# myfavouritekk/vdetlib

Measured on AMD Instinct MI355X. Metric: boxes/sec whole-node (NMS+temporal-conv+link), 300f×10k-box synth; mAP parity, higher is better.
Workload: dtype f32; 1 GPU; configs[1]+[2]: 1 video/GPU, 300 frames x 10000 boxes x 200 classes; per-(frame,class) NMS thresh 0.30 + temporal max-pool w=3 + 3-tap temporal convolution; greedy tubelets: 10 tracks/class (stop < 0.90), IoU-link >= 0.50, spatial max-pool IoU > 0.70 + completion + temporal max-pool; frames=300, boxes=10000, classes=200, scores=rand, parallelism=video-per-gpu x1, 4 distinct videos in flight per GPU

## Files before the change

### vdetlib_amd/csrc/adjrows_kernels.hpp

```cpp
#pragma once
#include <hip/hip_runtime.h>
#include <stdint.h>

#include "nms_kernels.hpp"
#include "binsort_kernels.hpp"

namespace vdet {

constexpr int kRowsChunk = 16;
constexpr int kRowsStage = 8192;
constexpr int kRowsStride = 72;

__global__ __launch_bounds__(256) void strip_totals_kernel(const GroupDesc *__restrict__ groups, const TileDesc *__restrict__ tiles,
                                                           int nstrips, const uint32_t *__restrict__ row_deg,
                                                           const uint32_t *__restrict__ group_flags, uint32_t *__restrict__ totals)
{
    const int lane = threadIdx.x & 63;
    const int sidx = blockIdx.x * 4 + (int)(threadIdx.x >> 6);
    if (sidx >= nstrips) return;
    const TileDesc td = tiles[sidx >> 2];
    const GroupDesc gd = groups[td.group];
    const int v = (td.row_tile * (kRowsPerTile / 64) + (sidx & 3)) * 64 + lane;
    uint32_t t = 0u;
    if ((group_flags[td.group] & kFlagRegular) && v < gd.nbox) t = (row_deg[gd.box_off + v] + 7u) & ~7u;
// ... 116 lines not shown
    const uint32_t total = s_total;
    const bool staged = total <= (uint32_t)kRowsStage;
    uint16_t *slab = adj + s_base;
    constexpr int kRowsSuper = 4 * kRowsChunk;
    for (int s0 = 0; s0 < ne; s0 += kRowsSuper) {
        unsigned long long mw[4 * WPW];
        uint16_t xw[4 * WPW];
#pragma unroll
        for (int j = 0; j < 4 * WPW; ++j) {
            const int q = j / WPW, i = j % WPW;
            const int c = (int)scol[min(s0 + kRowsChunk * q + w + 4 * i, ne - 1)];
            mw[j] = gbits[bit_word(B, min(v, B - 1), c)];
            xw[j] = tr[min(c * 64 + lane, B - 1)];
        }
#pragma unroll
        for (int q = 0; q < 4; ++q) {
            const int e0 = s0 + kRowsChunk * q;
            if (e0 >= ne) break;
#pragma unroll
            for (int i = 0; i < WPW; ++i) {
                const int el = w + 4 * i;
                sb[el * kRowsStride + lane] = (e0 + el < ne && v < B) ? mw[q * WPW + i] : 0ull;
                sx[el * 64 + lane] = xw[q * WPW + i];
            }
            lds_only_barrier();
#pragma unroll 1
            for (int i = 0; i < kRowsChunk / 4; ++i) {
                const int el = 4 * i + xa;
                unsigned long long m = sb[el * kRowsStride + xrow];
                const uint32_t cnt = (uint32_t)__popcll(m);
                if (__ballot(cnt != 0u) == 0ull) continue;
                const uint16_t *sxw = sx + el * 64;
                uint32_t pos = 0u;
                if (cnt != 0u) {
                    const uint32_t at = atomicAdd(&scur[xrow], cnt);
                    if (at == 0u) spad[xrow] = sxw[__ffsll(m) - 1];
                    pos = my_off + at;
                }
                if (staged) {
                    while (__ballot(m != 0ull) != 0ull) {
                        if (m != 0ull) {
                            const unsigned long long m1 = m & (m - 1ull);
                            const uint16_t v0 = sxw[__ffsll(m) - 1];
                            const uint16_t v1 = sxw[m1 ? __ffsll(m1) - 1 : 0];
                            sstage[pos] = v0;
                            if (m1) sstage[pos + 1] = v1;
                            pos += m1 ? 2u : 1u;
                            m = m1 & (m1 - 1ull);
                        }
                    }
                } else {
                    while (__ballot(m != 0ull) != 0ull) {
                        if (m != 0ull) {
                            slab[pos++] = sxw[__ffsll(m) - 1];
                            m &= m - 1ull;
                        }
                    }
                }
            }
            lds_only_barrier();
        }
    }
    __syncthreads();
    if (tid < 64) {
        const uint32_t deg = srow_deg[tid];
        const uint32_t p = srow_off[tid] + deg, padv = spad[tid];
        const uint32_t npad = ((deg + 7u) & ~7u) - deg;
        if (deg != 0u)
            for (uint32_t k = 0; k < npad; ++k) { if (staged) sstage[p + k] = (uint16_t)padv; else slab[p + k] = (uint16_t)padv; }
    }
    if (staged) {
        __syncthreads();
        const uint4 *s4 = reinterpret_cast<const uint4 *>(sstage);
        uint4 *d4 = reinterpret_cast<uint4 *>(slab);
        for (uint32_t i = tid; i < (total >> 3); i += 256) d4[i] = s4[i];
    }
}

__global__ __launch_bounds__(256) void adj_finish_kernel(const GroupDesc *__restrict__ groups, const TileDesc *__restrict__ tiles,
                                                         const uint32_t *__restrict__ row_deg, uint2 *__restrict__ row_meta,
                                                         uint16_t *__restrict__ adj, uint32_t slot_cap, int *__restrict__ status,
                                                         const uint32_t *__restrict__ group_flags, const float4 *__restrict__ xbox_all,
                                                         const uint16_t *__restrict__ xord_all, int over_bits,
                                                         WalkMeta *__restrict__ wmeta, uint4 *__restrict__ wmeta16)
{
    const TileDesc td = tiles[blockIdx.x];
    const uint32_t gf = group_flags[td.group];
    if (!(gf & kFlagRegular)) return;
    const GroupDesc gd = groups[td.group];
    const int v = td.row_tile * kRowsPerTile + (int)threadIdx.x;
    if (v >= gd.nbox) return;
    const uint32_t row = (uint32_t)(gd.box_off + v);
    const uint32_t deg = row_deg[row];
    const int vo = (int)xord_all[row];
    const float4 bx = xbox_all[row];
    const bool over = deg > slot_cap;
    if (over) atomicOr(status, over_bits);
    const uint32_t p = over ? 0u : row * slot_cap;
    const uint32_t d = over ? 0u : deg;
    if (d & 7u) {
        uint16_t *l = adj + (uint64_t)p;
        for (uint32_t k = d; k < ((d + 7u) & ~7u); ++k) l[k] = (uint16_t)vo;
    }
    row_meta[gd.box_off + vo] = make_uint2(p, d);
    const bool rec16 = wmeta16 && (gf & kFlagU16);
    if (wmeta && !rec16) {
        wmeta[gd.box_off + vo].box = over ? make_float4(0.f, 0.f, 0.f, 0.f) : bx;
        wmeta[gd.box_off + vo].row = make_uint4(p, d, 0u, 0u);
    }
    if (rec16)
        wmeta16[gd.box_off + vo] = over ? make_uint4(0u, 0u, 0u, 0u)
                                        : make_uint4((uint32_t)bx.x | ((uint32_t)bx.y << 16), (uint32_t)bx.z | ((uint32_t)bx.w << 16), p, d);
}

__global__ __launch_bounds__(256) void deg_sum_kernel(const uint32_t *__restrict__ row_deg, int64_t n, unsigned long long *__restrict__ out)
{
    unsigned long long s = 0ull;
    for (int64_t i = (int64_t)blockIdx.x * 256 + threadIdx.x; i < n; i += (int64_t)gridDim.x * 256) s += (row_deg[i] + 7u) & ~7u;
    for (int d = 32; d > 0; d >>= 1) s += __shfl_xor(s, d, 64);
    if ((threadIdx.x & 63) == 0 && s) atomicAdd(out, s);
}

__global__ void pool_start_kernel(unsigned long long *pool_used, unsigned long long first) { *pool_used = first; }

}
```

### vdetlib_amd/csrc/graphlists_kernels.hpp

```cpp
#pragma once
#include <hip/hip_runtime.h>
#include <stdint.h>

#include "nms_kernels.hpp"

namespace vdet {

__device__ __forceinline__ int qreach_slot(const GroupDesc &gd, int g) { return ((gd.box_off >> 8) + g) * 4; }

__global__ __launch_bounds__(256) void row_classes_kernel(const float4 *__restrict__ xbox, const GroupDesc *__restrict__ groups,
                                                          const uint32_t *__restrict__ group_flags, float one_minus_t,
                                                          uint16_t *__restrict__ rowperm, float *__restrict__ qreach)
{
    __shared__ float sw[256];
    __shared__ float sreach[256];
    const int g = blockIdx.x, t = blockIdx.y, tid = threadIdx.x;
    if (!(group_flags[g] & kFlagRegular)) return;
    const GroupDesc gd = groups[g];
    if (t * 256 >= gd.nbox) return;
    const int s = t * 256 + tid;
    const bool valid = s < gd.nbox;
    float wd = 3.0e38f, reach = -3.0e38f;
    if (valid) { const float4 b = xbox[gd.box_off + s]; wd = b.z - b.x; reach = b.x + one_minus_t * ((b.z - b.x) + 1.0f) * 1.001f + 1.0f; }
    sw[tid] = wd;
    __syncthreads();
    int rank = 0;
    for (int j = 0; j < 256; ++j) { const float o = sw[j]; rank += (o < wd || (o == wd && j < tid)) ? 1 : 0; }
    if (valid) rowperm[gd.box_off + t * 256 + rank] = (uint16_t)s;
    sreach[rank] = reach;
    __syncthreads();
    float rc = sreach[tid];
#pragma unroll
    for (int d = 32; d > 0; d >>= 1) rc = fmaxf(rc, __shfl_xor(rc, d, 64));
    if ((tid & 63) == 0) qreach[qreach_slot(gd, g) + 4 * t + (tid >> 6)] = rc;
}

struct ListItem { int32_t group; int32_t tq; };

struct GraphListsParams {
    const float4 *xbox;
    const uint16_t *xord;
    const GroupDesc *groups;
    const uint32_t *group_flags;
    const ListItem *items;
    int nitems;
    float t32, hg, one_minus_t;
    uint32_t *row_deg;
    const float2 *reach_table;
    const uint16_t *rowperm;
    const float *qreach;
    uint16_t *adj;
    uint32_t slot_cap;
    int *status;
    int over_bits;
    uint32_t trash_off;
};

__device__ __forceinline__ void emit_half(uint16_t *__restrict__ adj, uint32_t h, uint32_t boff, const uint16_t *ids, uint32_t *lpos,
                                          const uint16_t myid)
{
    constexpr int kSlots = 4;
    if (__ballot(h != 0u) == 0ull) return;
    uint32_t hk[kSlots];
    uint16_t ek[kSlots];
    int bk[kSlots];
#pragma unroll
    for (int k = 0; k < kSlots; ++k) { hk[k] = h; bk[k] = __builtin_ctz(h | 0x80000000u); h &= h - 1u; }
#pragma unroll
    for (int k = 0; k < kSlots; ++k) ek[k] = ids[bk[k]];
#pragma unroll
    for (int k = 0; k < kSlots; ++k) {
        if (hk[k] != 0u) {
            *reinterpret_cast<uint16_t *>(reinterpret_cast<char *>(adj) + (boff + 2u * k)) = ek[k];
            const uint32_t o = __hip_atomic_fetch_add(&lpos[bk[k]], 2u, __ATOMIC_RELAXED, __HIP_MEMORY_SCOPE_WAVEFRONT);
            *reinterpret_cast<uint16_t *>(reinterpret_cast<char *>(adj) + o) = myid;
        }
    }
    boff += 2u * kSlots;
    while (__ballot(h != 0u) != 0ull) {
        if (h != 0u) {
            const int b = __builtin_ctz(h);
            *reinterpret_cast<uint16_t *>(reinterpret_cast<char *>(adj) + boff) = ids[b];
            const uint32_t o = __hip_atomic_fetch_add(&lpos[b], 2u, __ATOMIC_RELAXED, __HIP_MEMORY_SCOPE_WAVEFRONT);
            *reinterpret_cast<uint16_t *>(reinterpret_cast<char *>(adj) + o) = myid;
            boff += 2u;
            h &= h - 1u;
        }
    }
}

__device__ __forceinline__ void emit_block(const uint32_t slot_cap, uint16_t *__restrict__ adj, int *__restrict__ status, const int over_bits,
                                           const uint32_t trash_off, unsigned long long m, const uint32_t tcnt, const uint32_t pat,
                                           const uint32_t ptat, const uint32_t row_slot, const uint32_t col_slot, const uint16_t *cids,
                                           const uint16_t myid, uint32_t *lpos, const int lane)
{
    const uint32_t cnt = (uint32_t)__popcll(m);
    const bool rover = pat + cnt > slot_cap, cover = ptat + tcnt > slot_cap;
    if ((rover && cnt) || (cover && tcnt)) atomicOr(status, over_bits);
    lpos[lane] = cover ? trash_off : (col_slot * slot_cap + ptat) * 2u;
    const uint32_t boff = rover ? trash_off : (row_slot * slot_cap + pat) * 2u;
    emit_half(adj, (uint32_t)m, boff, cids, lpos, myid);
    emit_half(adj, (uint32_t)(m >> 32), boff + 2u * (uint32_t)__popc((uint32_t)m), cids + 32, lpos + 32, myid);
}

template <bool XS, bool INTS>
__device__ __forceinline__ void margin_block(const float4 brx, const float rarea, const float4 *sb, const float *sa, float t32, float hg,
                                             uint32_t &lo, uint32_t &hi)
{
    uint32_t nr0 = 0, nr1 = 0;
#pragma unroll 1
    for (int g = 0; g < 4; ++g) {
#pragma unroll
        for (int j = 0; j < 8; ++j) {
            const int k = 31 - 8 * g - j;
// ... 119 lines not shown
```

### vdetlib_amd/csrc/nms_kernels.hpp

```cpp
#pragma once
#include <hip/hip_runtime.h>
#include <stdint.h>

namespace vdet {

struct GroupDesc {
    int32_t box_off;
    int32_t nbox;
    int64_t bits_off;
};

__device__ __host__ __forceinline__ int64_t bit_word(int nbox, int v, int c)
{
    const int W = (nbox + 63) >> 6;
    return ((int64_t)(v >> 6) * W + c) * 64 + (v & 63);
}
__host__ __device__ __forceinline__ int64_t bit_words_of_group(int nbox)
{
    const int64_t W = (nbox + 63) >> 6;
    return W * W * 64;
}

struct TileDesc {
    int32_t group;
// ... 64 lines not shown
    if (group_flags && (group_flags[td.group] & kFlagRegular)) return;
    const GroupDesc gd = groups[td.group];
    const int B = gd.nbox;
    const int tid = threadIdx.x;
    const int v = td.row_tile * kRowsPerTile + tid;
    const int W = (B + 63) >> 6;
    int wper = (W + gridDim.y - 1) / gridDim.y;
    wper = (wper + 3) & ~3;
    const int w0 = blockIdx.y * wper;
    const int w1 = min(W, w0 + wper);
    if (w0 >= w1) return;

    const float qnan = __uint_as_float(0x7FC00000u);
    float4 brow = make_float4(qnan, qnan, qnan, qnan);
    if (v < B) brow = boxes[gd.box_off + v];
    const float rarea = box_area(brow);
    uint32_t zcnt = 0;

    for (int wt = w0; wt < w1; wt += 4) {
        __syncthreads();
        {
            const int u = wt * 64 + tid;
            float4 bi = make_float4(qnan, qnan, qnan, qnan);
            if (u < B) bi = boxes[gd.box_off + u];
            sbox[tid] = bi;
            sarea[tid] = box_area(bi);
        }
        __syncthreads();
        const int nw = min(4, w1 - wt);
        for (int q = 0; q < nw; ++q) {
            uint32_t lo = 0, hi = 0;
#pragma unroll
            for (int k = 0; k < 32; ++k) {
                const uint32_t p = pair_pred(brow, rarea, sbox[q * 64 + k], sarea[q * 64 + k], t32);
                lo |= (p & 1u) << k;
                zcnt += p >> 1;
            }
#pragma unroll
            for (int k = 0; k < 32; ++k) {
                const uint32_t p = pair_pred(brow, rarea, sbox[q * 64 + 32 + k], sarea[q * 64 + 32 + k], t32);
                hi |= (p & 1u) << k;
                zcnt += p >> 1;
            }
            uint64_t m = ((uint64_t)hi << 32) | lo;
            const int cbase = (wt + q) * 64;
            if (v >= cbase && v < cbase + 64) {
                m &= ~(1ull << (v - cbase));
                const uint32_t ps = pair_pred(brow, rarea, brow, rarea, t32);
                zcnt -= ps >> 1;
            }
            if (v < B) bits[gd.bits_off + bit_word(B, v, wt + q)] = m;
        }
    }
    if (v < B && zcnt) {
        atomicAdd(&row_z[gd.box_off + v], zcnt);
        group_z[td.group] = 1u;
    }
}

struct FrameIndex {
    const float4 *xbox;
    const uint16_t *xord;
    const uint32_t *cum;
    const float *info;
    const uint2 *xbox16;
    const uint16_t *xord16;
    int64_t bias16;
};

__device__ __host__ __forceinline__ int64_t pair_pos(int64_t box_off_plus_g) { return (box_off_plus_g + 1) & ~(int64_t)1; }

__device__ __forceinline__ int xbucket(float x, float xmin, float scale)
{
    const float t = (x - xmin) * scale;
    return t <= 0.0f ? 0 : (t >= 255.0f ? 255 : (int)t);
}

__global__ void xkey_kernel(const float4 *__restrict__ boxes, uint32_t *__restrict__ keys, int64_t n)
{
    const int64_t i = (int64_t)blockIdx.x * blockDim.x + threadIdx.x;
    if (i < n) keys[i] = ~score_key(boxes[i].x);
}

__global__ __launch_bounds__(256) void frame_index_kernel(const float4 *__restrict__ boxes, const GroupDesc *__restrict__ groups,
                                                          const uint16_t *__restrict__ xord_all, float4 *__restrict__ xbox_all,
                                                          uint32_t *__restrict__ cum, float *__restrict__ info,
                                                          const uint32_t *__restrict__ group_flags, uint2 *__restrict__ xbox16,
                                                          uint16_t *__restrict__ xord16)
{
    __shared__ float smin[256], smax[256], swm[256];
    __shared__ uint32_t hist[257];
    const int f = blockIdx.x, tid = threadIdx.x;
    const int B = groups[f].nbox;
    const int64_t fo = groups[f].box_off;
    const float4 *fb = boxes + fo;
    const uint16_t *xord = xord_all + fo;
    float4 *xbox = xbox_all + fo;
    float mn = 3.0e38f, mx = -3.0e38f, wm = 0.0f;
    const bool u16 = xbox16 && (group_flags[f] & kFlagU16);
    const int64_t p16 = pair_pos(fo + f);
    for (int r = tid; r < B; r += 256) {
        const uint16_t o = xord[r];
        const float4 b = fb[o];
        xbox[r] = b;
        if (u16) {
            xbox16[p16 + r] = make_uint2((uint32_t)b.x | ((uint32_t)b.y << 16), (uint32_t)b.z | ((uint32_t)b.w << 16));
            xord16[p16 + r] = o;
        }
        mn = fminf(mn, b.x); mx = fmaxf(mx, b.x); wm = fmaxf(wm, (b.z - b.x) + 1.0f);
    }
    smin[tid] = mn; smax[tid] = mx; swm[tid] = wm;
    for (int i = tid; i < 257; i += 256) hist[i] = 0;
    __syncthreads();
    for (int d = 128; d > 0; d >>= 1) {
        if (tid < d) { smin[tid] = fminf(smin[tid], smin[tid + d]); smax[tid] = fmaxf(smax[tid], smax[tid + d]); swm[tid] = fmaxf(swm[tid], swm[tid + d]); }
        __syncthreads();
    }
    const float xmin = smin[0], xmax = smax[0];
    const float scale = xmax > xmin ? 256.0f / (xmax - xmin) : 0.0f;
    for (int r = tid; r < B; r += 256) atomicAdd(&hist[xbucket(fb[r].x, xmin, scale) + 1], 1u);
    __syncthreads();
    if (tid == 0) {
        uint32_t run = 0;
        for (int k = 0; k <= 256; ++k) { run += hist[k]; cum[(int64_t)f * 257 + k] = run; }
        info[f * 4 + 0] = xmin; info[f * 4 + 1] = scale; info[f * 4 + 2] = swm[0]; info[f * 4 + 3] = 0.0f;
    }
}

__device__ __forceinline__ void xwindow(const FrameIndex &ix, int f, float x1c, float wc, double t, int &r0, int &r1)
{
    const float xmin = ix.info[f * 4 + 0], scale = ix.info[f * 4 + 1], wmax = ix.info[f * 4 + 2];
    const double wj = fmin((double)wmax, (double)wc / t * 1.001);
    const double lo = (double)x1c - (1.0 - t) * wj * 1.001 - 1.0;
    const double hi = (double)x1c + (1.0 - t) * (double)wc * 1.001 + 1.0;
    const int b0 = xbucket((float)fmax(lo, -3.0e38), xmin, scale);
    const int b1 = xbucket((float)fmin(hi, 3.0e38), xmin, scale);
    r0 = (int)ix.cum[(int64_t)f * 257 + b0];
    r1 = (int)ix.cum[(int64_t)f * 257 + b1 + 1];
}

constexpr float kRegularCoordMax = 1152921504606846976.0f;
__global__ __launch_bounds__(256) void frame_flags_kernel(const float4 *__restrict__ boxes,
                                                          const GroupDesc *__restrict__ groups,
                                                          uint32_t *__restrict__ group_flags,
                                                          int *__restrict__ n_irregular)
{
    const GroupDesc gd = groups[blockIdx.x];
    int bad = 0, wide = 0;
    const float inf = __uint_as_float(0x7F800000u);
    for (int v = threadIdx.x; v < gd.nbox; v += 256) {
        const float4 b = boxes[gd.box_off + v];
        const float w = (b.z - b.x) + 1.0f, h = (b.w - b.y) + 1.0f;
        const float a = w * h;
        const bool ok = fabsf(b.x) <= kRegularCoordMax && fabsf(b.y) <= kRegularCoordMax && fabsf(b.z) <= kRegularCoordMax &&
                        fabsf(b.w) <= kRegularCoordMax && w > 0.0f && h > 0.0f && a < inf;
        bad |= ok ? 0 : 1;
        const bool small = b.x == truncf(b.x) && b.y == truncf(b.y) && b.z == truncf(b.z) && b.w == truncf(b.w) &&
                           fmaxf(fmaxf(b.x, b.y), fmaxf(b.z, b.w)) <= 65535.0f &&
                           ((__float_as_uint(b.x) | __float_as_uint(b.y) | __float_as_uint(b.z) | __float_as_uint(b.w)) >> 31) == 0u;
        wide |= small ? 0 : 1;
    }
    const int any_bad = __syncthreads_or(bad);
    const int any_wide = __syncthreads_or(wide);
    if (threadIdx.x == 0) {
        group_flags[blockIdx.x] = (any_bad ? 0u : kFlagRegular) | (any_wide ? 0u : kFlagU16);
        if (any_bad) atomicAdd(n_irregular, 1);
    }
}

__device__ __attribute__((noinline)) bool pair_pred_exact_slow(float4 bi, float iarea, float4 bj, float jarea, float t32)
{
    return (pair_pred(bi, iarea, bj, jarea, t32) & 1u) != 0;
}

struct TilePair {
    int32_t group;
    int16_t rt, ct;
};

__device__ __forceinline__ float amax(float a, float b) { float r; asm("v_max_f32 %0, %1, %2" : "=v"(r) : "v"(a), "v"(b)); return r; }
__device__ __forceinline__ float amin(float a, float b) { float r; asm("v_min_f32 %0, %1, %2" : "=v"(r) : "v"(a), "v"(b)); return r; }

template <bool XSORTED = false>
__device__ __forceinline__ bool pred_regular(float4 br, float rarea, float4 bc, float carea, float t32, float t32e,
                                             bool &border)
{
    const float xx1 = XSORTED ? bc.x : amax(br.x, bc.x);
    const float yy1 = amax(br.y, bc.y);
    const float xx2 = amin(br.z, bc.z);
    const float yy2 = amin(br.w, bc.w);
    const float w = amax(0.0f, (xx2 - xx1) + 1.0f);
    const float h = (yy2 - yy1) + 1.0f;
    const float inter = w * h;
    const float uni = (rarea + carea) - inter;
    const float r = __builtin_fmaf(-t32, uni, inter);
    const float bnd = t32e * uni;
    const bool p = r >= 0.0f;
    border = !p && (r >= -bnd);
    return p;
}

__device__ __forceinline__ void shl1_or_sign(uint32_t &acc, float v)
{
    acc = __builtin_amdgcn_alignbit(acc, __float_as_uint(v), 31);
}

template <bool XSORTED, bool INTS>
// ... 1400 lines not shown
```

### vdetlib_amd/csrc/vdet_capi.hip

```cpp
#include <hip/hip_runtime.h>
#include <atomic>
#include <chrono>

#include <algorithm>
#include <cmath>
#include <cstdarg>
#include <cstdio>
#include <cstdlib>
#include <cstring>
#include <initializer_list>
#include <string>
#include <vector>

#include "../../include/vdet_hip.h"
#include "nms_kernels.hpp"
#include "binsort_kernels.hpp"
#include "small_kernels.hpp"
#include "detnms_kernels.hpp"
#include "fused_kernels.hpp"
#include "adjrows_kernels.hpp"
#include "graphlists_kernels.hpp"
#include "temporal_kernels.hpp"
#include "tubelet_kernels.hpp"
#include "track_kernels.hpp"
// ... 354 lines not shown
    while (p < x) p <<= 1;
    return p;
}

int translate_status(vdet_ctx *c, int st)
{
    if (st & kStPoolAsync) return fail(c, VDET_EAGAIN, "adjacency pool overflow in an asynchronous graph build: run the calls again");
    if (st & kStBadOrder) return fail(c, VDET_EINVAL, "a caller-supplied candidate list holds a count or a box index out of range");
    if (st & kStBadAnchor) return fail(c, VDET_EINVAL, "an anchor frame lies outside the video");
    if (st & kStBadPixAnchor) return fail(c, VDET_EINVAL, "track_pixels: an anchor frame outside the video, or an anchor box that is not finite, beyond 2^20, empty or wholly outside the image (the slot is written as an empty one)");
    if (st & kStBadMerge) return fail(c, VDET_EINVAL, "merge 'max': two paired tubelets differ in the frames of their boxes or in their anchor frame");
    if (st & kStBadPropagate) return fail(c, VDET_EINVAL, "propagate_boxes: a keep_cnt outside 0..cap, a keep_idx outside 0..B-1, or a source box that is not finite or beyond 2^20 (the source writes NaN rows)");
    if (st & kStBadKeep) return fail(c, VDET_EINVAL, "nms_tracks: a keep_cnt outside 0..cap or a keep_idx outside 0..B-1 (the entry is skipped)");
    if (st & kStPatchCap) return fail(c, VDET_ECAP, "tubelet_patches / tubelet_rois: more present tubelet boxes in the frame range than cap (the first cap windows are valid)");
    if (st & kStSvmBad) return fail(c, VDET_EINVAL, "svm_head: a slot row outside shape or a class column outside W (the group is skipped, nothing is written for it)");
    if (st & kStEvalList) return fail(c, VDET_EINVAL, "a keep list holds a NaN score, an increasing score or a count / box index out of range");
    if (st & kStDivZero) return fail(c, VDET_EDIVZERO, "float division (zero union)");
    if (st & kStCap) return fail(c, VDET_ECAP, "more survivors than the output capacity");
    if (st & kStPool) return fail(c, VDET_EHIP, "internal: adjacency pool overflow");
    return VDET_OK;
}

int make_plan(vdet_ctx *c, NmsPlan &pl)
{
    const size_t budget_words = std::max<size_t>(c->bits_budget / 8, 1);
    size_t cur = 0;
    int t0 = 0, p0 = 0, d0 = 0;
    pl.nmax = 0;
    pl.ntot = 0;
    for (size_t g = 0; g < pl.groups.size(); ++g) {
        GroupDesc &gd = pl.groups[g];
        pl.ntot = std::max<int64_t>(pl.ntot, (int64_t)gd.box_off + gd.nbox);
        pl.nmax = std::max(pl.nmax, gd.nbox);
        if (gd.nbox < 2) { gd.bits_off = 0; continue; }
        const size_t words = (size_t)bit_words_of_group(gd.nbox);
        if (cur && cur + words > budget_words) {
            pl.batch_tiles.push_back({t0, (int)pl.tiles.size()});
            pl.batch_pairs.push_back({p0, (int)pl.pairs.size()});
            pl.batch_ditems.push_back({d0, (int)pl.ditems.size()});
            t0 = (int)pl.tiles.size();
            p0 = (int)pl.pairs.size();
            d0 = (int)pl.ditems.size();
            pl.bits_words_max = std::max(pl.bits_words_max, cur);
            cur = 0;
        }
        gd.bits_off = (int64_t)cur;
        cur += words;
        const int nrt = (gd.nbox + kRowsPerTile - 1) / kRowsPerTile;
        for (int rt = 0; rt < nrt; ++rt) pl.tiles.push_back({(int32_t)g, rt});
        for (int rt = 0; rt < nrt; ++rt)
            for (int ct = rt; ct < nrt; ++ct) pl.pairs.push_back({(int32_t)g, (int16_t)rt, (int16_t)ct});
        for (int q = 3; q >= 0; --q)
            for (int rt = 0; rt < nrt; ++rt) pl.ditems.push_back({(int32_t)g, (int32_t)(4 * rt + q)});
    }
    if ((int)pl.tiles.size() > t0) {
        pl.batch_tiles.push_back({t0, (int)pl.tiles.size()});
        pl.batch_pairs.push_back({p0, (int)pl.pairs.size()});
        pl.batch_ditems.push_back({d0, (int)pl.ditems.size()});
    }
    pl.bits_words_max = std::max(pl.bits_words_max, cur);
    (void)c;
    return VDET_OK;
}

int sort_groups_by_keys(vdet_ctx *c, int G, int nmax, int64_t ntot);

int build_frame_index(vdet_ctx *c, const float4 *d_boxes, int64_t ntot, int64_t G, int nmax)
{
    if (c->cache_enabled && c->index_valid && c->index_boxes == d_boxes && c->index_F == G && c->index_B == ntot) return VDET_OK;
    c->index_valid = false;
    HIPCHK(c, c->xkeys.reserve((size_t)ntot * 4));
    HIPCHK(c, c->xord.reserve((size_t)ntot * 2));
    HIPCHK(c, c->xncand.reserve((size_t)G * 4));
    HIPCHK(c, c->xbox.reserve((size_t)ntot * 16));
    HIPCHK(c, c->xbox16.reserve((size_t)(ntot + G + 4) * 8));
    HIPCHK(c, c->xord16.reserve((size_t)(ntot + G + 4) * 2));
    HIPCHK(c, c->xcum.reserve((size_t)G * 257 * 4));
    HIPCHK(c, c->xinfo.reserve((size_t)G * 16));
    StageTimer tm(c, ST_OTHER);
    hipLaunchKernelGGL(xkey_kernel, dim3((unsigned)((ntot + 255) / 256)), dim3(256), 0, c->stream, d_boxes,
                       c->xkeys.as<uint32_t>(), ntot);
    int rc = sort_groups_by_keys(c, (int)G, nmax, ntot);
    if (rc) return rc;
    hipLaunchKernelGGL(frame_index_kernel, dim3((unsigned)G), dim3(256), 0, c->stream, d_boxes, c->groups.as<GroupDesc>(),
                       c->xord.as<uint16_t>(), c->xbox.as<float4>(), c->xcum.as<uint32_t>(), c->xinfo.as<float>(),
                       c->gflags.as<uint32_t>(), c->xbox16.as<uint2>(), c->xord16.as<uint16_t>());
    HIPCHK(c, hipGetLastError());
    c->index_valid = true; c->index_boxes = d_boxes; c->index_F = G; c->index_B = ntot;
    return VDET_OK;
}

FrameIndex frame_index_of(vdet_ctx *c)
{
    return FrameIndex{c->xbox.as<float4>(), c->xord.as<uint16_t>(), c->xcum.as<uint32_t>(), c->xinfo.as<float>(),
                      c->xbox16.as<uint2>(), c->xord16.as<uint16_t>(), 0};
}

NmsPlan &volume_plan(vdet_ctx *c, int64_t F, int64_t B)
{
    if (c->vplan_F == F && c->vplan_B == B && c->vplan_budget == c->bits_budget && !c->vplan.groups.empty()) return c->vplan;
    (void)host_sync(c);
    c->graph_valid = c->lists_valid = c->index_valid = c->nodes_valid = false;
    c->vplan = NmsPlan();
    c->vplan.groups.resize((size_t)F);
    for (int64_t f = 0; f < F; ++f) c->vplan.groups[(size_t)f] = {(int32_t)(f * B), (int32_t)B, 0};
    make_plan(c, c->vplan);
    c->vplan_F = F; c->vplan_B = B; c->vplan_budget = c->bits_budget;
    c->vplan_valid = false;
    return c->vplan;
}

int volume_groups(vdet_ctx *c, int64_t F, int64_t B)
{
    NmsPlan &pl = volume_plan(c, F, B);
    c->host_groups = &pl.groups;
    HIPCHK(c, c->groups.reserve((size_t)F * sizeof(GroupDesc)));
    if (!c->vplan_valid)
        HIPCHK(c, hipMemcpyAsync(c->groups.p, pl.groups.data(), (size_t)F * sizeof(GroupDesc), hipMemcpyHostToDevice, c->stream));
    return VDET_OK;
}

int build_graph(vdet_ctx *c, const float4 *d_boxes, NmsPlan &pl, float t32, double thresh, bool volume);

int ensure_volume_graph(vdet_ctx *c, const float *d_boxes, int64_t F, int64_t B, double nms_thres, bool reuse, bool *reused = nullptr)
{
    const float t32 = thresh_to_f32(nms_thres);
    const bool same = reuse && c->cache_enabled && c->graph_valid && c->prep.boxes == d_boxes && c->prep.F == F && c->prep.B == B &&
                      memcmp(&c->prep.t32, &t32, 4) == 0;
    if (reused) *reused = same;
    if (same) return VDET_OK;
    c->graph_valid = c->lists_valid = c->nodes_valid = false;
    const int rc = build_graph(c, reinterpret_cast<const float4 *>(d_boxes), volume_plan(c, F, B), t32, nms_thres, true);
    if (rc) return rc;
    c->prep.boxes = d_boxes; c->prep.F = F; c->prep.B = B; c->prep.t32 = t32;
    c->graph_valid = true;
    return VDET_OK;
}

bool lists_match(const vdet_ctx *c, const ListsKey &key, int64_t F, int64_t B) { return c->lists_valid && c->prep.F == F && c->prep.B == B && c->prep.lists == key; }
void set_lists(vdet_ctx *c, const ListsKey &key) { c->prep.lists = key; c->lists_valid = true; }

bool index_matches(const vdet_ctx *c, const float *d_boxes, int64_t F, int64_t B)
{
    return c->cache_enabled && c->graph_valid && c->index_valid && c->prep.boxes == d_boxes && c->prep.F == F && c->prep.B == B && c->index_boxes == d_boxes;
}

bool nodes_match(const vdet_ctx *c, const float *d_tracks, const float *d_boxes, int64_t F, int64_t B, int64_t C, int T)
{
    const float nt = thresh_to_f32(c->nodekey.nms_thres);
    return c->cache_enabled && c->nodes_valid && c->graph_valid && c->nodekey.tracks == d_tracks && c->nodekey.boxes == d_boxes &&
           c->prep.boxes == d_boxes && c->nodekey.F == F && c->nodekey.B == B && c->nodekey.C == C && c->nodekey.T == T &&
           c->prep.F == F && c->prep.B == B && memcmp(&c->prep.t32, &nt, 4) == 0;
}

bool rescore_from_graph(const uint32_t *group_flags, double nms_thres, double overlap_thres)
{
    return group_flags && overlap_thres - nms_thres > 0.05 && nms_thres > 0.0 && overlap_thres < 1.0;
}

struct TrackWork {
    const uint32_t *flags;
    FrameIndex ix;
    bool filled;
    float link_t32;
    int reach, mask_words, lazy;
    bool need_suppress;
};
// ... 139 lines not shown
                hipLaunchKernelGGL(frame_flags_kernel, dim3((unsigned)G), dim3(256), 0, c->stream, d_boxes,
                                   c->groups.as<GroupDesc>(), c->gflags.as<uint32_t>(), &c->d_cnt->irregular);
            }
            if (!volume) c->index_valid = false;
            const int rci = build_frame_index(c, d_boxes, pl.ntot, (int64_t)G, pl.nmax);
            if (rci) return rci;
            HIPCHK(c, c->reachtab.reserve((size_t)(pl.ntot / 64 + (int64_t)G + 2) * sizeof(float2)));
            {
                StageTimer tm(c, ST_OTHER);
                hipLaunchKernelGGL(reach_table_kernel, dim3((unsigned)G), dim3(256), 0, c->stream, c->xbox.as<float4>(),
                                   c->groups.as<GroupDesc>(), c->gflags.as<uint32_t>(), one_minus_t, c->reachtab.as<float2>());
                if (direct) {
                    HIPCHK(c, c->rowperm.reserve((size_t)pl.ntot * 2 + 1024));
                    HIPCHK(c, c->qreach.reserve((size_t)(pl.ntot / 256 + (int64_t)G + 2) * 4 * sizeof(float)));
                    hipLaunchKernelGGL(row_classes_kernel, dim3((unsigned)G, (unsigned)((pl.nmax + 255) / 256)), dim3(256), 0, c->stream,
                                       c->xbox.as<float4>(), c->groups.as<GroupDesc>(), c->gflags.as<uint32_t>(), one_minus_t,
                                       c->rowperm.as<uint16_t>(), c->qreach.as<float>());
                }
            }
        } else {
            c->index_valid = false;
        }
        if (direct && !pl.ditems.empty()) {
            StageTimer tm(c, ST_IOU_BITS);
            GraphListsParams gp;
            gp.xbox = c->xbox.as<float4>(); gp.xord = c->xord.as<uint16_t>(); gp.groups = c->groups.as<GroupDesc>();
            gp.group_flags = c->gflags.as<uint32_t>(); gp.items = c->ditems.as<ListItem>(); gp.nitems = (int)pl.ditems.size();
            gp.t32 = t32; gp.hg = half_gap(t32); gp.one_minus_t = one_minus_t; gp.row_deg = c->rowz.as<uint32_t>(); gp.reach_table = c->reachtab.as<float2>();
            gp.rowperm = c->rowperm.as<uint16_t>(); gp.qreach = c->qreach.as<float>(); gp.adj = c->adj.as<uint16_t>();
            gp.slot_cap = c->direct_cap; gp.status = &c->d_cnt->status; gp.over_bits = pool_bits | kStDirect;
            gp.trash_off = (uint32_t)((unsigned long long)pl.ntot * c->direct_cap * 2ull);
            hipLaunchKernelGGL(graph_lists_kernel, dim3((gp.nitems + 7) & ~7), dim3(64), 0, c->stream, gp);
        }
        for (size_t bi = 0; bi < pl.batch_tiles.size(); ++bi) {
            const auto bt = pl.batch_tiles[bi];
            const auto bp = pl.batch_pairs[bi];
            const int nt = bt.second - bt.first;
            if (nt <= 0) continue;
            uint64_t *bits_b = c->bits.as<uint64_t>();
            if (use_sym && !direct && bp.second > bp.first) {
                StageTimer tm(c, ST_IOU_BITS);
                if (c->wave_transpose)
                    hipLaunchKernelGGL(iou_bits_sym_kernel<true>, dim3(bp.second - bp.first), dim3(256), 0, c->stream,
                                       c->xbox.as<float4>(), c->groups.as<GroupDesc>(), c->gflags.as<uint32_t>(),
                                       c->pairs.as<TilePair>() + bp.first, t32, half_gap(t32), one_minus_t, bits_b, c->rowz.as<uint32_t>(),
                                       c->reachtab.as<float2>());
                else
                    hipLaunchKernelGGL(iou_bits_sym_kernel<false>, dim3(bp.second - bp.first), dim3(256), 0, c->stream,
                                       c->xbox.as<float4>(), c->groups.as<GroupDesc>(), c->gflags.as<uint32_t>(),
                                       c->pairs.as<TilePair>() + bp.first, t32, half_gap(t32), one_minus_t, bits_b, c->rowz.as<uint32_t>(),
                                       c->reachtab.as<float2>());
            }
            int splits = 1;
            if (nt < 4 * c->n_cu) {
                int wmax = 1;
                for (int t = bt.first; t < bt.second; ++t)
                    wmax = std::max(wmax, (pl.groups[pl.tiles[t].group].nbox + 63) / 64);
                splits = std::min((4 * c->n_cu + nt - 1) / nt, (wmax + 3) / 4);
                splits = std::max(1, std::min(splits, 65535));
            }
            {
                StageTimer tm(c, ST_IOU_GEN);
                hipLaunchKernelGGL(iou_bits_kernel, dim3(nt, splits), dim3(256), 0, c->stream, d_boxes,
                                   c->groups.as<GroupDesc>(), c->tiles.as<TileDesc>() + bt.first, t32,
                                   bits_b, c->rowz.as<uint32_t>(), c->groupz.as<uint32_t>(),
                                   use_sym ? c->gflags.as<uint32_t>() : (const uint32_t *)nullptr);
            }
            {
                StageTimer tm(c, ST_ADJ);
                const bool k2_tile = pl.nmax <= 384;
                const bool rows_path = use_sym && c->adj_rows && !k2_tile;
                hipLaunchKernelGGL(k2_tile ? adj_build_kernel<kRowsPerTile> : adj_build_kernel<kAdjRows>, dim3(k2_tile ? nt : 2 * nt),
                                   dim3(k2_tile ? kRowsPerTile : kAdjRows), 0, c->stream, d_boxes,
                                   c->groups.as<GroupDesc>(), c->tiles.as<TileDesc>() + bt.first,
                                   bits_b, c->rowz.as<uint32_t>(), c->rowmeta.as<uint2>(),
                                   c->adj.as<uint16_t>(), &c->d_cnt->pool_used, pool_cap,
                                   &c->d_cnt->status, use_sym ? c->gflags.as<uint32_t>() : (const uint32_t *)nullptr,
                                   use_sym ? frame_index_of(c) : FrameIndex{}, one_minus_t,
                                   async ? (kStPool | kStPoolAsync) : kStPool,
                                   c->wmeta_built ? c->wmeta.as<WalkMeta>() : (WalkMeta *)nullptr,
                                   use_sym ? c->reachtab.as<float2>() : (const float2 *)nullptr, rows_path ? 1 : 0);
                if (rows_path && direct) {
                    if (bi == 0)
                    hipLaunchKernelGGL(adj_finish_kernel, dim3((unsigned)pl.tiles.size()), dim3(256), 0, c->stream, c->groups.as<GroupDesc>(),
                                       c->tiles.as<TileDesc>(), c->rowz.as<uint32_t>(), c->rowmeta.as<uint2>(),
                                       c->adj.as<uint16_t>(), c->direct_cap, &c->d_cnt->status, c->gflags.as<uint32_t>(),
                                       c->xbox.as<float4>(), c->xord.as<uint16_t>(), pool_bits | kStDirect,
                                       c->wmeta_built ? c->wmeta.as<WalkMeta>() : (WalkMeta *)nullptr,
                                       c->wmeta_built ? c->wmeta16.as<uint4>() : (uint4 *)nullptr);
                    c->wmeta16_built = c->wmeta_built;
                } else if (rows_path) {
                    HIPCHK(c, c->striptot.reserve((size_t)4 * nt * 4));
                    HIPCHK(c, c->stripoff.reserve((size_t)4 * nt * 8));
                    hipLaunchKernelGGL(strip_totals_kernel, dim3(nt), dim3(256), 0, c->stream, c->groups.as<GroupDesc>(),
                                       c->tiles.as<TileDesc>() + bt.first, 4 * nt, c->rowz.as<uint32_t>(), c->gflags.as<uint32_t>(),
                                       c->striptot.as<uint32_t>());
                    hipLaunchKernelGGL(strip_scan_kernel, dim3(1), dim3(1024), 0, c->stream, c->striptot.as<uint32_t>(), 4 * nt,
                                       c->stripoff.as<unsigned long long>(), &c->d_cnt->pool_used);
                    hipLaunchKernelGGL(adj_rows_kernel, dim3(4 * nt), dim3(256), 0, c->stream, c->groups.as<GroupDesc>(),
                                       c->tiles.as<TileDesc>() + bt.first, bits_b, c->rowz.as<uint32_t>(), c->rowmeta.as<uint2>(),
                                       c->adj.as<uint16_t>(), c->stripoff.as<unsigned long long>(), pool_cap, &c->d_cnt->status, c->gflags.as<uint32_t>(),
                                       c->xbox.as<float4>(), c->xord.as<uint16_t>(), async ? (kStPool | kStPoolAsync) : kStPool,
                                       c->wmeta_built ? c->wmeta.as<WalkMeta>() : (WalkMeta *)nullptr, c->reachtab.as<float2>(),
                                       c->wmeta_built ? c->wmeta16.as<uint4>() : (uint4 *)nullptr);
                    c->wmeta16_built = c->wmeta_built;
                }
            }
        }
        HIPCHK(c, hipGetLastError());
        if (async) {
            c->all_regular = false;
            return VDET_OK;
        }
        Counters h;
        HIPCHK(c, hipMemcpyAsync(&h, c->d_cnt, sizeof h, hipMemcpyDeviceToHost, c->stream));
        HIPCHK(c, host_sync(c));
        c->all_regular = use_sym && h.irregular == 0;
        if (!(h.status & kStPool)) {
            c->pool_hint = std::max(c->pool_hint, h.pool_used);
            return VDET_OK;
        }
        if (h.status & kStDirect) {
            c->direct_lists = false;
            continue;
        }
        if (h.pool_used > 0xFFFFFFFFull) return fail(c, VDET_ENOMEM, "suppression graph has more than 2^32 edges");
        if (attempt == 2) break;
        HIPCHK(c, c->adj.reserve((size_t)h.pool_used * 2 + 4096));
    }
    return fail(c, VDET_EHIP, "internal: adjacency pool overflow after regrow");
}

struct SortWalkArgs {
    bool sort_only = false;
    bool walk_only = false;
    uint16_t *order_out = nullptr;
    int32_t *ncand_out = nullptr;
    const uint16_t *order_in = nullptr;
    const int32_t *ncand_in = nullptr;
    int mode, P, B, C;
    const float *scores;
    const uint32_t *keys;
    const uint8_t *excl;
    int use_thr;
    float thr;
    int topk = 0;
    int32_t *nover_out = nullptr;
    int32_t *keep_idx;
    int32_t *keep_cnt;
    int64_t cap;
};

SortWalkArgs volume_sort_args(int64_t F, int64_t B, int64_t C, const float *d_scores)
{
    SortWalkArgs a{};
    a.sort_only = true;
    a.mode = 0; a.P = (int)(F * C); a.B = (int)B; a.C = (int)C;
    a.scores = d_scores;
    return a;
}

SortWalkArgs volume_walk_args(int64_t F, int64_t B, int64_t C, const float *d_scores, int32_t *keep_idx, int32_t *keep_cnt, int64_t cap)
{
    SortWalkArgs a = volume_sort_args(F, B, C, d_scores);
    a.sort_only = false;
    a.walk_only = true;
    a.keep_idx = keep_idx; a.keep_cnt = keep_cnt; a.cap = cap;
    return a;
}

int sort_comp_desc(vdet_ctx *c, uint32_t n);

// ... 3916 lines not shown
```

Baseline: 367.3 million boxes/s.

## Bitonic-sort row classes, parallel histogram scan, wider frame index, swizzled adj finish

Swaps the O(n^2) rank-counting sort in row_classes_kernel for a 256-wide bitonic sort on packed (width, slot) keys, done mostly with wave shuffles plus a few LDS exchanges. frame_index_kernel becomes templated on block size, uses 1024 threads for large frames, and replaces the serial single-thread histogram prefix sum with a wave-shuffle scan. adj_finish_kernel remaps block indices across eight interleaved groups and writes the row padding with vectorised 2/4/8-byte stores instead of a byte loop. A standalone check program is added for the new rowperm ordering; edge cases such as -0.0 width and invalid slots now depend on the key encoding.

```diff
diff --git a/devtools/rowperm_check.hip b/devtools/rowperm_check.hip
--- /dev/null
+++ b/devtools/rowperm_check.hip
@@ -0,0 +1,101 @@
+#include <hip/hip_runtime.h>
+
+#include <cmath>
+#include <cstdio>
+#include <cstring>
+#include <random>
+#include <vector>
+
+#include "../vdetlib_amd/csrc/graphlists_kernels.hpp"
+
+#define CHK(x) do { hipError_t e_ = (x); if (e_ != hipSuccess) { printf("%s: %s\n", #x, hipGetErrorString(e_)); return 2; } } while (0)
+
+int main()
+{
+    using namespace vdet;
+    const int sizes[] = {385, 256, 257, 1025, 1, 129, 10000, 450, 64, 511, 512, 513, 300, 2000};
+    const int G = (int)(sizeof sizes / sizeof sizes[0]);
+    const int irregular = 8;
+    std::mt19937 rng(4402);
+    std::vector<GroupDesc> groups((size_t)G);
+    std::vector<uint32_t> flags((size_t)G, kFlagRegular);
+    flags[irregular] = 0u;
+    int ntot = 0, nmax = 0;
+    for (int g = 0; g < G; ++g) { groups[g] = GroupDesc{}; groups[g].box_off = ntot; groups[g].nbox = sizes[g]; ntot += sizes[g]; nmax = std::max(nmax, sizes[g]); }
+    std::vector<float4> xbox((size_t)ntot);
+    const float special[] = {0.0f, -0.0f, 7.0f, -0.5f, 3.5f, 2305843009213693952.0f};
+    for (int g = 0; g < G; ++g) {
+        const int kind = g % 4;
+        for (int v = 0; v < sizes[g]; ++v) {
+            float w;
+            if (kind == 0) w = (float)(rng() % 6);
+            else if (kind == 1) w = (float)(rng() % 30000) / 100.0f - 0.9f;
+            else if (kind == 2) w = special[rng() % 6];
+            else w = 120.0f;
+            float x1 = (float)(rng() % 1200);
+            float x2 = x1 + w;
+            if (w == 2305843009213693952.0f) { x1 = -1152921504606846976.0f; x2 = 1152921504606846976.0f; }
+            if (w == 0.0f && std::signbit(w)) { x1 = 0.0f; x2 = -0.0f; }
+            xbox[groups[g].box_off + v] = make_float4(x1, (float)(rng() % 700), x2, 800.0f);
+        }
+    }
+    const float one_minus_t = 0.7f;
+    const size_t nperm = (size_t)ntot + 512, nq = (size_t)(ntot / 256 + G + 2) * 4;
+    std::vector<uint16_t> want_perm(nperm, 0xFFFFu);
+    std::vector<uint32_t> want_q(nq, 0xFFFFFFFFu);
+    for (int g = 0; g < G; ++g) {
+        if (!(flags[g] & kFlagRegular)) continue;
+        const GroupDesc gd = groups[g];
+        for (int t = 0; t * 256 < gd.nbox; ++t) {
+            float wd[256], reach[256], byrank[256];
+            bool valid[256];
+            for (int i = 0; i < 256; ++i) {
+                const int s = t * 256 + i;
+                valid[i] = s < gd.nbox;
+                wd[i] = 0.0f; reach[i] = -3.0e38f;
+                if (valid[i]) { const float4 b = xbox[gd.box_off + s]; wd[i] = b.z - b.x; reach[i] = b.x + one_minus_t * ((b.z - b.x) + 1.0f) * 1.001f + 1.0f; }
+            }
+            for (int i = 0; i < 256; ++i) {
+                int rank = 0;
+                for (int j = 0; j < 256; ++j) {
+                    bool before;
+                    if (valid[i] != valid[j]) before = valid[j];
+                    else if (!valid[i]) before = j < i;
+                    else before = wd[j] < wd[i] || (wd[j] == wd[i] && j < i);
+                    rank += before ? 1 : 0;
+                }
+                if (valid[i]) want_perm[gd.box_off + t * 256 + rank] = (uint16_t)(t * 256 + i);
+                byrank[rank] = reach[i];
+            }
+            for (int q = 0; q < 4; ++q) {
+                float m = byrank[64 * q];
+                for (int i = 1; i < 64; ++i) m = fmaxf(m, byrank[64 * q + i]);
+                memcpy(&want_q[((gd.box_off >> 8) + g) * 4 + 4 * t + q], &m, 4);
+            }
+        }
+    }
+    float4 *d_xbox; GroupDesc *d_groups; uint32_t *d_flags; uint16_t *d_perm; float *d_q;
+    CHK(hipMalloc(&d_xbox, xbox.size() * sizeof(float4)));
+    CHK(hipMalloc(&d_groups, groups.size() * sizeof(GroupDesc)));
+    CHK(hipMalloc(&d_flags, flags.size() * 4));
+    CHK(hipMalloc(&d_perm, nperm * 2));
+    CHK(hipMalloc(&d_q, nq * 4));
+    CHK(hipMemcpy(d_xbox, xbox.data(), xbox.size() * sizeof(float4), hipMemcpyHostToDevice));
+    CHK(hipMemcpy(d_groups, groups.data(), groups.size() * sizeof(GroupDesc), hipMemcpyHostToDevice));
+    CHK(hipMemcpy(d_flags, flags.data(), flags.size() * 4, hipMemcpyHostToDevice));
+    CHK(hipMemset(d_perm, 0xFF, nperm * 2));
+    CHK(hipMemset(d_q, 0xFF, nq * 4));
+    hipLaunchKernelGGL(row_classes_kernel, dim3((unsigned)G, (unsigned)((nmax + 255) / 256)), dim3(256), 0, 0, d_xbox, d_groups, d_flags,
+                       one_minus_t, d_perm, d_q);
+    CHK(hipGetLastError());
+    CHK(hipDeviceSynchronize());
+    std::vector<uint16_t> got_perm(nperm);
+    std::vector<uint32_t> got_q(nq);
+    CHK(hipMemcpy(got_perm.data(), d_perm, nperm * 2, hipMemcpyDeviceToHost));
+    CHK(hipMemcpy(got_q.data(), d_q, nq * 4, hipMemcpyDeviceToHost));
+    size_t bad_perm = 0, bad_q = 0;
+    for (size_t i = 0; i < nperm; ++i) bad_perm += got_perm[i] != want_perm[i];
+    for (size_t i = 0; i < nq; ++i) bad_q += got_q[i] != want_q[i];
+    printf("rowperm_check: %d frames, %d boxes; rowperm %zu of %zu differ, qreach %zu of %zu differ\n", G, ntot, bad_perm, nperm, bad_q, nq);
+    return (bad_perm || bad_q) ? 1 : 0;
+}
diff --git a/vdetlib_amd/csrc/adjrows_kernels.hpp b/vdetlib_amd/csrc/adjrows_kernels.hpp
--- a/vdetlib_amd/csrc/adjrows_kernels.hpp
+++ b/vdetlib_amd/csrc/adjrows_kernels.hpp
@@ -222,9 +222,12 @@
                                                          uint16_t *__restrict__ adj, uint32_t slot_cap, int *__restrict__ status,
                                                          const uint32_t *__restrict__ group_flags, const float4 *__restrict__ xbox_all,
                                                          const uint16_t *__restrict__ xord_all, int over_bits,
-                                                         WalkMeta *__restrict__ wmeta, uint4 *__restrict__ wmeta16)
-{
-    const TileDesc td = tiles[blockIdx.x];
+                                                         WalkMeta *__restrict__ wmeta, uint4 *__restrict__ wmeta16, uint32_t ntiles)
+{
+    const uint32_t per = gridDim.x >> 3;
+    const uint32_t tile = (blockIdx.x & 7u) * per + (blockIdx.x >> 3);
+    if (tile >= ntiles) return;
+    const TileDesc td = tiles[tile];
     const uint32_t gf = group_flags[td.group];
     if (!(gf & kFlagRegular)) return;
     const GroupDesc gd = groups[td.group];
@@ -238,9 +241,13 @@
     if (over) atomicOr(status, over_bits);
     const uint32_t p = over ? 0u : row * slot_cap;
     const uint32_t d = over ? 0u : deg;
-    if (d & 7u) {
-        uint16_t *l = adj + (uint64_t)p;
-        for (uint32_t k = d; k < ((d + 7u) & ~7u); ++k) l[k] = (uint16_t)vo;
+    {
+        char *l = reinterpret_cast<char *>(adj + (uint64_t)p);
+        const uint32_t v2 = (uint32_t)vo | ((uint32_t)vo << 16);
+        uint32_t k = d;
+        if (k & 1u) { *reinterpret_cast<uint16_t *>(l + 2u * k) = (uint16_t)vo; k += 1u; }
+        if (k & 2u) { *reinterpret_cast<uint32_t *>(l + 2u * k) = v2; k += 2u; }
+        if (k & 4u) { *reinterpret_cast<uint2 *>(l + 2u * k) = make_uint2(v2, v2); }
     }
     row_meta[gd.box_off + vo] = make_uint2(p, d);
     const bool rec16 = wmeta16 && (gf & kFlagU16);
diff --git a/vdetlib_amd/csrc/graphlists_kernels.hpp b/vdetlib_amd/csrc/graphlists_kernels.hpp
--- a/vdetlib_amd/csrc/graphlists_kernels.hpp
+++ b/vdetlib_amd/csrc/graphlists_kernels.hpp
@@ -8,11 +8,50 @@
 
 __device__ __forceinline__ int qreach_slot(const GroupDesc &gd, int g) { return ((gd.box_off >> 8) + g) * 4; }
 
+__device__ __forceinline__ unsigned long long rank_key(const bool valid, float wd, const int slot)
+{
+    wd = wd == 0.0f ? 0.0f : wd;
+    const uint32_t u = __float_as_uint(wd);
+    const uint32_t m = valid ? (u ^ ((u >> 31) ? 0xFFFFFFFFu : 0x80000000u)) : 0xFFFFFFFFu;
+    return ((unsigned long long)m << 8) | (unsigned long long)slot;
+}
+
+template <int K, int J>
+__device__ __forceinline__ unsigned long long bitonic_pick(const unsigned long long key, const unsigned long long other, const int tid)
+{
+    const bool keep_min = ((tid & J) == 0) == ((tid & K) == 0);
+    const bool other_less = other < key;
+    return (other_less == keep_min) ? other : key;
+}
+
+template <int K, int J>
+__device__ __forceinline__ unsigned long long bitonic_lane_step(const unsigned long long key, const int tid)
+{
+    static_assert(J < 64, "partners of a lane exchange sit in one wave");
+    return bitonic_pick<K, J>(key, __shfl_xor(key, J, 64), tid);
+}
+
+template <int K, int J>
+__device__ __forceinline__ unsigned long long bitonic_lds_step(const unsigned long long key, unsigned long long *buf, const int tid)
+{
+    buf[tid] = key;
+    __syncthreads();
+    return bitonic_pick<K, J>(key, buf[tid ^ J], tid);
+}
+
+template <int K>
+__device__ __forceinline__ unsigned long long bitonic_lane_tail(unsigned long long key, const int tid)
+{
+    key = bitonic_lane_step<K, 32>(key, tid); key = bitonic_lane_step<K, 16>(key, tid); key = bitonic_lane_step<K, 8>(key, tid);
+    key = bitonic_lane_step<K, 4>(key, tid);  key = bitonic_lane_step<K, 2>(key, tid);  key = bitonic_lane_step<K, 1>(key, tid);
+    return key;
+}
+
 __global__ __launch_bounds__(256) void row_classes_kernel(const float4 *__restrict__ xbox, const GroupDesc *__restrict__ groups,
                                                           const uint32_t *__restrict__ group_flags, float one_minus_t,
                                                           uint16_t *__restrict__ rowperm, float *__restrict__ qreach)
 {
-    __shared__ float sw[256];
+    __shared__ unsigned long long skey[2][256];
     __shared__ float sreach[256];
     const int g = blockIdx.x, t = blockIdx.y, tid = threadIdx.x;
     if (!(group_flags[g] & kFlagRegular)) return;
@@ -20,16 +59,26 @@
     if (t * 256 >= gd.nbox) return;
     const int s = t * 256 + tid;
     const bool valid = s < gd.nbox;
-    float wd = 3.0e38f, reach = -3.0e38f;
+    float wd = 0.0f, reach = -3.0e38f;
     if (valid) { const float4 b = xbox[gd.box_off + s]; wd = b.z - b.x; reach = b.x + one_minus_t * ((b.z - b.x) + 1.0f) * 1.001f + 1.0f; }
-    sw[tid] = wd;
-    __syncthreads();
-    int rank = 0;
-    for (int j = 0; j < 256; ++j) { const float o = sw[j]; rank += (o < wd || (o == wd && j < tid)) ? 1 : 0; }
-    if (valid) rowperm[gd.box_off + t * 256 + rank] = (uint16_t)s;
-    sreach[rank] = reach;
-    __syncthreads();
-    float rc = sreach[tid];
+    sreach[tid] = reach;
+    unsigned long long key = rank_key(valid, wd, tid);
+    key = bitonic_lane_step<2, 1>(key, tid);
+    key = bitonic_lane_step<4, 2>(key, tid);   key = bitonic_lane_step<4, 1>(key, tid);
+    key = bitonic_lane_step<8, 4>(key, tid);   key = bitonic_lane_step<8, 2>(key, tid);   key = bitonic_lane_step<8, 1>(key, tid);
+    key = bitonic_lane_step<16, 8>(key, tid);  key = bitonic_lane_step<16, 4>(key, tid);  key = bitonic_lane_step<16, 2>(key, tid);
+    key = bitonic_lane_step<16, 1>(key, tid);
+    key = bitonic_lane_step<32, 16>(key, tid); key = bitonic_lane_step<32, 8>(key, tid);  key = bitonic_lane_step<32, 4>(key, tid);
+    key = bitonic_lane_step<32, 2>(key, tid);  key = bitonic_lane_step<32, 1>(key, tid);
+    key = bitonic_lane_tail<64>(key, tid);
+    key = bitonic_lds_step<128, 64>(key, skey[0], tid);
+    key = bitonic_lane_tail<128>(key, tid);
+    key = bitonic_lds_step<256, 128>(key, skey[1], tid);
+    key = bitonic_lds_step<256, 64>(key, skey[0], tid);
+    key = bitonic_lane_tail<256>(key, tid);
+    const int src = (int)(key & 0xFFull);
+    if (t * 256 + src < gd.nbox) rowperm[gd.box_off + s] = (uint16_t)(t * 256 + src);
+    float rc = sreach[src];
 #pragma unroll
     for (int d = 32; d > 0; d >>= 1) rc = fmaxf(rc, __shfl_xor(rc, d, 64));
     if ((tid & 63) == 0) qreach[qreach_slot(gd, g) + 4 * t + (tid >> 6)] = rc;
diff --git a/vdetlib_amd/csrc/nms_kernels.hpp b/vdetlib_amd/csrc/nms_kernels.hpp
--- a/vdetlib_amd/csrc/nms_kernels.hpp
+++ b/vdetlib_amd/csrc/nms_kernels.hpp
@@ -170,14 +170,15 @@
     if (i < n) keys[i] = ~score_key(boxes[i].x);
 }
 
-__global__ __launch_bounds__(256) void frame_index_kernel(const float4 *__restrict__ boxes, const GroupDesc *__restrict__ groups,
+template <int NT>
+__global__ __launch_bounds__(NT) void frame_index_kernel(const float4 *__restrict__ boxes, const GroupDesc *__restrict__ groups,
                                                           const uint16_t *__restrict__ xord_all, float4 *__restrict__ xbox_all,
                                                           uint32_t *__restrict__ cum, float *__restrict__ info,
                                                           const uint32_t *__restrict__ group_flags, uint2 *__restrict__ xbox16,
                                                           uint16_t *__restrict__ xord16)
 {
-    __shared__ float smin[256], smax[256], swm[256];
-    __shared__ uint32_t hist[257];
+    __shared__ float smin[NT], smax[NT], swm[NT];
+    __shared__ uint32_t hist[257], wsum[4];
     const int f = blockIdx.x, tid = threadIdx.x;
     const int B = groups[f].nbox;
     const int64_t fo = groups[f].box_off;
@@ -187,7 +188,7 @@
     float mn = 3.0e38f, mx = -3.0e38f, wm = 0.0f;
     const bool u16 = xbox16 && (group_flags[f] & kFlagU16);
     const int64_t p16 = pair_pos(fo + f);
-    for (int r = tid; r < B; r += 256) {
+    for (int r = tid; r < B; r += NT) {
         const uint16_t o = xord[r];
         const float4 b = fb[o];
         xbox[r] = b;
@@ -198,19 +199,30 @@
         mn = fminf(mn, b.x); mx = fmaxf(mx, b.x); wm = fmaxf(wm, (b.z - b.x) + 1.0f);
     }
     smin[tid] = mn; smax[tid] = mx; swm[tid] = wm;
-    for (int i = tid; i < 257; i += 256) hist[i] = 0;
+    for (int i = tid; i < 257; i += NT) hist[i] = 0;
     __syncthreads();
-    for (int d = 128; d > 0; d >>= 1) {
+    for (int d = NT / 2; d > 0; d >>= 1) {
         if (tid < d) { smin[tid] = fminf(smin[tid], smin[tid + d]); smax[tid] = fmaxf(smax[tid], smax[tid + d]); swm[tid] = fmaxf(swm[tid], swm[tid + d]); }
         __syncthreads();
     }
     const float xmin = smin[0], xmax = smax[0];
     const float scale = xmax > xmin ? 256.0f / (xmax - xmin) : 0.0f;
-    for (int r = tid; r < B; r += 256) atomicAdd(&hist[xbucket(fb[r].x, xmin, scale) + 1], 1u);
+    for (int r = tid; r < B; r += NT) atomicAdd(&hist[xbucket(fb[r].x, xmin, scale) + 1], 1u);
     __syncthreads();
+    uint32_t incl = 0u;
+    if (tid < 256) {
+        incl = hist[tid + 1];
+#pragma unroll
+        for (int d = 1; d < 64; d <<= 1) { const uint32_t o = __shfl_up(incl, d, 64); if ((tid & 63) >= d) incl += o; }
+        if ((tid & 63) == 63) wsum[tid >> 6] = incl;
+    }
+    __syncthreads();
+    if (tid < 256) {
+        for (int w = 0; w < (tid >> 6); ++w) incl += wsum[w];
+        cum[(int64_t)f * 257 + tid + 1] = incl;
+    }
     if (tid == 0) {
-        uint32_t run = 0;
-        for (int k = 0; k <= 256; ++k) { run += hist[k]; cum[(int64_t)f * 257 + k] = run; }
+        cum[(int64_t)f * 257] = 0u;
         info[f * 4 + 0] = xmin; info[f * 4 + 1] = scale; info[f * 4 + 2] = swm[0]; info[f * 4 + 3] = 0.0f;
     }
 }
diff --git a/vdetlib_amd/csrc/vdet_capi.hip b/vdetlib_amd/csrc/vdet_capi.hip
--- a/vdetlib_amd/csrc/vdet_capi.hip
+++ b/vdetlib_amd/csrc/vdet_capi.hip
@@ -460,7 +460,7 @@
                        c->xkeys.as<uint32_t>(), ntot);
     int rc = sort_groups_by_keys(c, (int)G, nmax, ntot);
     if (rc) return rc;
-    hipLaunchKernelGGL(frame_index_kernel, dim3((unsigned)G), dim3(256), 0, c->stream, d_boxes, c->groups.as<GroupDesc>(),
+    hipLaunchKernelGGL(nmax > 1024 ? frame_index_kernel<1024> : frame_index_kernel<256>, dim3((unsigned)G), dim3(nmax > 1024 ? 1024 : 256), 0, c->stream, d_boxes, c->groups.as<GroupDesc>(),
                        c->xord.as<uint16_t>(), c->xbox.as<float4>(), c->xcum.as<uint32_t>(), c->xinfo.as<float>(),
                        c->gflags.as<uint32_t>(), c->xbox16.as<uint2>(), c->xord16.as<uint16_t>());
     HIPCHK(c, hipGetLastError());
@@ -766,12 +766,12 @@
                                    use_sym ? c->reachtab.as<float2>() : (const float2 *)nullptr, rows_path ? 1 : 0);
                 if (rows_path && direct) {
                     if (bi == 0)
-                    hipLaunchKernelGGL(adj_finish_kernel, dim3((unsigned)pl.tiles.size()), dim3(256), 0, c->stream, c->groups.as<GroupDesc>(),
+                    hipLaunchKernelGGL(adj_finish_kernel, dim3((unsigned)((pl.tiles.size() + 7) & ~(size_t)7)), dim3(256), 0, c->stream, c->groups.as<GroupDesc>(),
                                        c->tiles.as<TileDesc>(), c->rowz.as<uint32_t>(), c->rowmeta.as<uint2>(),
                                        c->adj.as<uint16_t>(), c->direct_cap, &c->d_cnt->status, c->gflags.as<uint32_t>(),
                                        c->xbox.as<float4>(), c->xord.as<uint16_t>(), pool_bits | kStDirect,
                                        c->wmeta_built ? c->wmeta.as<WalkMeta>() : (WalkMeta *)nullptr,
-                                       c->wmeta_built ? c->wmeta16.as<uint4>() : (uint4 *)nullptr);
+                                       c->wmeta_built ? c->wmeta16.as<uint4>() : (uint4 *)nullptr, (uint32_t)pl.tiles.size());
                     c->wmeta16_built = c->wmeta_built;
                 } else if (rows_path) {
                     HIPCHK(c, c->striptot.reserve((size_t)4 * nt * 4));
```

After: 371.9 million boxes/s (median of 6 runs). 1.01x the previous value.
